# xswang/xflow

Hardware: NVIDIA H100
Metric: training examples/sec (higher is better)
Workload: dtype f32

## Files before the change

xflow_b200/csrc/kernels.cu:

```cuda
#include <cuda_runtime.h>
#include <stdint.h>
#include <stdlib.h>

#include "kernels.h"
#include "table.cuh"

__global__ void xf_k_fill(uint8_t* base, uint64_t cap, uint32_t stride, int lazy) {
  const uint64_t chunks_per_row = stride / 16;
  const uint64_t total = cap * chunks_per_row;
  for (uint64_t c = (uint64_t)blockIdx.x * blockDim.x + threadIdx.x; c < total;
       c += (uint64_t)gridDim.x * blockDim.x) {
    uint64_t r = c / chunks_per_row;
    uint32_t q = (uint32_t)(c % chunks_per_row);
    uint4 v = make_uint4(0, 0, 0, 0);
    if (q == 0) {
      v.x = 0xFFFFFFFFu; v.y = 0xFFFFFFFFu;
      if (!lazy) v.w = XF_NEG_ZERO_BITS;
    }
    *reinterpret_cast<uint4*>(base + r * stride + (uint64_t)q * 16) = v;
  }
}

template <int VEC>
__device__ __forceinline__ void xf_ldv(const float* p, float (&o)[VEC]) {
  if (VEC == 4) { float4 t = __ldcg(reinterpret_cast<const float4*>(p)); o[0] = t.x; o[1 % VEC] = t.y; o[2 % VEC] = t.z; o[3 % VEC] = t.w; }
  else if (VEC == 2) { float2 t = __ldcg(reinterpret_cast<const float2*>(p)); o[0] = t.x; o[1 % VEC] = t.y; }
  else { o[0] = __ldcg(p); }
}
template <int VEC>
__device__ __forceinline__ void xf_stv(float* p, const float (&o)[VEC]) {
  if (VEC == 4) *reinterpret_cast<float4*>(p) = make_float4(o[0], o[1 % VEC], o[2 % VEC], o[3 % VEC]);
  else if (VEC == 2) *reinterpret_cast<float2*>(p) = make_float2(o[0], o[1 % VEC]);
  else *p = o[0];
}
template <int VEC, bool SLOTG, bool STAMP>
__global__ void __launch_bounds__(256)
xf_k_update(XfTableView t, const uint32_t* __restrict__ slots, uint64_t n, int tps, double rows,
            const float* __restrict__ gw, const float* __restrict__ gv, int part,
            unsigned long long* __restrict__ live_total, const uint32_t* __restrict__ n_dev,
            const uint32_t* __restrict__ rows_dev, uint32_t extra_base, uint32_t extra_n,
            const float* __restrict__ v0_side, XfStampView sv) {
  __shared__ unsigned int s_live;
  if (threadIdx.x == 0) s_live = 0;
  __syncthreads();
  uint64_t n_head = n;
  if (n_dev != nullptr) {
    n_head = min((uint64_t)__ldg(n_dev), (uint64_t)extra_base);
    n = n_head + extra_n;
    rows = (double)__ldg(rows_dev);
  }
  unsigned int live_acc = 0;
  const int K = t.K;
  const unsigned lane = threadIdx.x & 31u;
  const uint64_t gwarp = ((uint64_t)blockIdx.x * blockDim.x + threadIdx.x) >> 5;
  const uint64_t nwarps = ((uint64_t)gridDim.x * blockDim.x) >> 5;
  const int q = (int)(lane & (unsigned)(tps - 1));
  const int gi = (int)(lane / (unsigned)tps);
  const int ngroups = 32 / tps;
  const int leader = (int)(lane & ~(unsigned)(tps - 1));
  const unsigned group_mask = (tps == 32) ? 0xffffffffu : (((1u << tps) - 1u) << leader);
  const int nchunk = K / VEC;

  for (uint64_t base = gwarp * 32; base < n; base += nwarps * 32) {
    const uint64_t e_fwd = base + lane;
    const uint64_t e_i = (SLOTG && e_fwd < n) ? (n - 1 - e_fwd) : e_fwd;
    const uint64_t e_phys = (e_i < n_head) ? e_i : (uint64_t)extra_base + (e_i - n_head);
    const uint32_t s_lane = (e_fwd < n) ? __ldcs(slots + e_phys) : 0xFFFFFFFFu;
    unsigned pend = __ballot_sync(0xffffffffu, s_lane != 0xFFFFFFFFu);
    if (live_total != nullptr && lane == 0) live_acc += __popc(pend);

    while (pend) {
      const int cnt = __popc(pend);
      const unsigned src = (gi < cnt) ? __fns(pend, 0, gi + 1) : 0u;
      const uint32_t s = __shfl_sync(0xffffffffu, s_lane, (int)src);
      const uint64_t i = __shfl_sync(0xffffffffu, (unsigned long long)e_i, (int)src);
      const uint64_t i_phys = __shfl_sync(0xffffffffu, (unsigned long long)e_phys, (int)src);
      uint8_t* rowp = (gi < cnt) ? xf_row(t, s) : nullptr;
      pend = (cnt <= ngroups) ? 0u : (pend & ~((2u << __fns(pend, 0, ngroups)) - 1u));

      const bool lat = K > 0 && (part & 2) && rowp != nullptr;
      float* vp = lat ? xf_row_v(rowp) : nullptr;
      float* nvp = lat ? xf_row_nv(rowp, K) : nullptr;
      float* zvp = lat ? xf_row_zv(rowp, K) : nullptr;
      float v0[VEC], n0[VEC], z0[VEC];
#pragma unroll
      for (int e = 0; e < VEC; ++e) { v0[e] = 0.f; n0[e] = 0.f; z0[e] = 0.f; }
      const bool has0 = lat && q < nchunk;
      if (has0) {
        xf_ldv<VEC>(vp + q * VEC, v0);
        if (t.opt == XF_OPT_FTRL) { xf_ldv<VEC>(nvp + q * VEC, n0); xf_ldv<VEC>(zvp + q * VEC, z0); }
      }
      float p0[VEC];
#pragma unroll
      for (int e = 0; e < VEC; ++e) p0[e] = 0.f;
      if (SLOTG && v0_side != nullptr && has0) {
        const uint64_t tok = (i_phys < (uint64_t)extra_base) ? i_phys : (uint64_t)__ldg(slots + i_phys + extra_n);
        xf_ldv<VEC>(v0_side + tok * (uint64_t)K + q * VEC, p0);
      }
      float ca0[VEC];
#pragma unroll
      for (int e = 0; e < VEC; ++e) ca0[e] = 0.f;
      if (SLOTG && t.canon && has0) xf_ldv<VEC>(xf_row_ca(t, rowp) + q * VEC, ca0);
      double accL = 0.0, accA = 0.0;
      if (SLOTG && has0) {
        const double2 a = __ldcg(reinterpret_cast<const double2*>(xf_row_acc(rowp, K)));
        accL = a.x;
        accA = a.y;
      }
      XfHead h;
      h.key = 0; h.flags = 0; h.w = h.n = h.z = 0.f; h.g = 0.0;
      if (q == 0 && rowp != nullptr) h = xf_load_head(rowp);
      const uint64_t key = __shfl_sync(group_mask, (unsigned long long)h.key, leader);
      const uint32_t flags = __shfl_sync(group_mask, h.flags, leader);
      if (rowp == nullptr) continue;

      if (q == 0) {
        if (!SLOTG) xf_apply_pending(t, h);
        if (part & 1) {
          const float g = SLOTG ? xf_div_rows((float)h.g, rows) : gw[i];
          xf_opt_coord(t, g, h.w, h.n, h.z);
        }
        if (SLOTG) h.g = -0.0;
        if (K > 0 && (part & 2)) h.flags |= XF_FLAG_V_READY;
        xf_store_head_t(t, rowp, h);
        if (STAMP) sv.stamp[s] = sv.now;
      }
      if (lat) {
        const bool ready = (flags & XF_FLAG_V_READY) != 0;
        for (int c = q; c < nchunk; c += tps) {
          const int k = c * VEC;
          float v[VEC], g[VEC], nn[VEC], zz[VEC];
#pragma unroll
          for (int e = 0; e < VEC; ++e) { v[e] = v0[e]; nn[e] = n0[e]; zz[e] = z0[e]; }
          if (c != q && ready) {
            xf_ldv<VEC>(vp + k, v);
            if (t.opt == XF_OPT_FTRL) { xf_ldv<VEC>(nvp + k, nn); xf_ldv<VEC>(zvp + k, zz); }
          }
          if (!ready) {
#pragma unroll
            for (int e = 0; e < VEC; ++e) { v[e] = xf_v_init(t, key, (uint32_t)(k + e)); nn[e] = 0.f; zz[e] = 0.f; }
          }
          if (SLOTG) {
            float vp0[VEC];
#pragma unroll
            for (int e = 0; e < VEC; ++e) vp0[e] = v[e];
            if (v0_side != nullptr) {
              if (c == q) {
#pragma unroll
                for (int e = 0; e < VEC; ++e) vp0[e] = p0[e];
              } else {
                const uint64_t tok = (i_phys < (uint64_t)extra_base) ? i_phys : (uint64_t)__ldg(slots + i_phys + extra_n);
                xf_ldv<VEC>(v0_side + tok * (uint64_t)K + k, vp0);
              }
            }
            if (t.canon) {
              float ca[VEC];
#pragma unroll
              for (int e = 0; e < VEC; ++e) ca[e] = ca0[e];
              if (c != q) xf_ldv<VEC>(xf_row_ca(t, rowp) + k, ca);
#pragma unroll
              for (int e = 0; e < VEC; ++e) g[e] = xf_div_rows((float)((double)ca[e] - (double)vp0[e] * accL), rows);
              const float zero[VEC] = {};
              xf_stv<VEC>(xf_row_ca(t, rowp) + k, zero);
            } else {
#pragma unroll
              for (int e = 0; e < VEC; ++e) g[e] = xf_div_rows((float)(accA - (double)vp0[e] * accL), rows);
            }
          } else {
#pragma unroll
            for (int e = 0; e < VEC; ++e) g[e] = gv[i * (uint64_t)K + k + e];
          }
          if (t.opt == XF_OPT_FTRL) {
#pragma unroll
            for (int e = 0; e < VEC; ++e) xf_ftrl_coord(t, g[e], v[e], nn[e], zz[e]);
            xf_stv<VEC>(nvp + k, nn);
            xf_stv<VEC>(zvp + k, zz);
          } else {
#pragma unroll
            for (int e = 0; e < VEC; ++e) xf_sgd_coord(t, g[e], v[e]);
          }
          xf_stv<VEC>(vp + k, v);
        }
        if (SLOTG) {
          __syncwarp(group_mask);
          if (q == 0) *reinterpret_cast<double2*>(xf_row_acc(rowp, K)) = make_double2(0.0, 0.0);
        }
      }
    }
  }
  if (live_total != nullptr) {
    if (lane == 0 && live_acc) atomicAdd(&s_live, live_acc);
    __syncthreads();
    if (threadIdx.x == 0 && s_live) atomicAdd_system(live_total, (unsigned long long)s_live);
  }
}

template <bool SLOTG>
__global__ void __launch_bounds__(256, 4)
xf_k_update_wide(XfTableView t, const uint32_t* __restrict__ slots, uint64_t n, int G, double rows,
                 const float* __restrict__ gw, const float* __restrict__ gv, int part,
                 unsigned long long* __restrict__ live_total, const uint32_t* __restrict__ n_dev,
                 const uint32_t* __restrict__ rows_dev, uint32_t extra_base, uint32_t extra_n,
                 const float* __restrict__ v0_side, XfStampView sv) {
  __shared__ unsigned int s_live;
  if (threadIdx.x == 0) s_live = 0;
  __syncthreads();
  uint64_t n_head = n;
  if (n_dev != nullptr) {
    n_head = min((uint64_t)__ldg(n_dev), (uint64_t)extra_base);
    n = n_head + extra_n;
    rows = (double)__ldg(rows_dev);
  }
  unsigned int live_acc = 0;
  const int K = t.K;
  const bool ftrl = t.opt == XF_OPT_FTRL;
  const int nV = K >> 2;
  const int units = (int)(t.stride >> 4);
  const int u_acc = 2 + nV, u_nv = u_acc + 1, u_zv = u_nv + nV;
  const unsigned lane = threadIdx.x & 31u;
  const uint64_t gwarp = ((uint64_t)blockIdx.x * blockDim.x + threadIdx.x) >> 5;
  const uint64_t nwarps = ((uint64_t)gridDim.x * blockDim.x) >> 5;
  const int q = (int)(lane & (unsigned)(G - 1));
  const int gi = (int)(lane / (unsigned)G);
  const int ngroups = 32 / G;
  const bool is_v = q >= 2 && q < 2 + nV;
  const int jv = q - 2;
  const int src_nv = is_v ? u_nv + jv : 0, src_zv = (is_v && ftrl) ? u_zv + jv : 0;
  const bool is_nv = ftrl && q >= u_nv && q < u_nv + nV, is_zv = ftrl && q >= u_zv && q < u_zv + nV;
  const int back = is_nv ? 2 + (q - u_nv) : (is_zv ? 2 + (q - u_zv) : 0);

  for (uint64_t base = gwarp * 32; base < n; base += nwarps * 32) {
    const uint64_t e_fwd = base + lane;
    const uint64_t e_i = (SLOTG && e_fwd < n) ? (n - 1 - e_fwd) : e_fwd;
    const uint64_t e_phys = (e_i < n_head) ? e_i : (uint64_t)extra_base + (e_i - n_head);
    const uint32_t s_lane = (e_fwd < n) ? __ldcs(slots + e_phys) : 0xFFFFFFFFu;
    unsigned pend = __ballot_sync(0xffffffffu, s_lane != 0xFFFFFFFFu);
    if (live_total != nullptr && lane == 0) live_acc += __popc(pend);
    while (pend) {
      const int cnt = __popc(pend);
      const unsigned src = (gi < cnt) ? __fns(pend, 0, gi + 1) : 0u;
      const uint32_t s = __shfl_sync(0xffffffffu, s_lane, (int)src);
      const uint64_t i = __shfl_sync(0xffffffffu, (unsigned long long)e_i, (int)src);
      const uint64_t i_phys = __shfl_sync(0xffffffffu, (unsigned long long)e_phys, (int)src);
      const bool live = gi < cnt;
      uint4* rowu = live ? reinterpret_cast<uint4*>(xf_row(t, s)) : nullptr;
      pend = (cnt <= ngroups) ? 0u : (pend & ~((2u << __fns(pend, 0, ngroups)) - 1u));

      uint4 u = make_uint4(0, 0, 0, 0);
      if (live && q < units) u = __ldcg(rowu + q);
      float4 side = make_float4(0.f, 0.f, 0.f, 0.f);
      if (live && is_v) {
        if (SLOTG) {
          if (v0_side != nullptr) {
            const uint64_t tok = (i_phys < (uint64_t)extra_base) ? i_phys : (uint64_t)__ldg(slots + i_phys + extra_n);
            side = __ldcg(reinterpret_cast<const float4*>(v0_side + tok * (uint64_t)K) + jv);
          }
        } else {
          side = __ldcg(reinterpret_cast<const float4*>(gv + i * (uint64_t)K) + jv);
        }
      }
      float gw_i = 0.f;
      if (!SLOTG && live && q == 1 && (part & 1)) gw_i = __ldg(gw + i);

      const uint32_t key_lo = __shfl_sync(0xffffffffu, u.x, 0, G), key_hi = __shfl_sync(0xffffffffu, u.y, 0, G);
      const uint32_t g_lo = __shfl_sync(0xffffffffu, u.z, 0, G), g_hi = __shfl_sync(0xffffffffu, u.w, 0, G);
      const uint32_t flags = __shfl_sync(0xffffffffu, u.w, 1, G);
      const uint32_t aL0 = __shfl_sync(0xffffffffu, u.x, u_acc, G), aL1 = __shfl_sync(0xffffffffu, u.y, u_acc, G);
      const uint32_t aA0 = __shfl_sync(0xffffffffu, u.z, u_acc, G), aA1 = __shfl_sync(0xffffffffu, u.w, u_acc, G);
      uint4 un, uz;
      un.x = __shfl_sync(0xffffffffu, u.x, src_nv, G); un.y = __shfl_sync(0xffffffffu, u.y, src_nv, G);
      un.z = __shfl_sync(0xffffffffu, u.z, src_nv, G); un.w = __shfl_sync(0xffffffffu, u.w, src_nv, G);
      uz.x = __shfl_sync(0xffffffffu, u.x, src_zv, G); uz.y = __shfl_sync(0xffffffffu, u.y, src_zv, G);
      uz.z = __shfl_sync(0xffffffffu, u.z, src_zv, G); uz.w = __shfl_sync(0xffffffffu, u.w, src_zv, G);
      const uint64_t key = (uint64_t)key_lo | ((uint64_t)key_hi << 32);
      const double g_acc = __longlong_as_double((long long)((uint64_t)g_lo | ((uint64_t)g_hi << 32)));
      const double accL = __longlong_as_double((long long)((uint64_t)aL0 | ((uint64_t)aL1 << 32)));
      const double accA = __longlong_as_double((long long)((uint64_t)aA0 | ((uint64_t)aA1 << 32)));
      const bool ready = (flags & XF_FLAG_V_READY) != 0;

      uint4 out = u;
      float nn[4] = {0.f, 0.f, 0.f, 0.f}, zz[4] = {0.f, 0.f, 0.f, 0.f};
      if (q == 0 && SLOTG) { out.z = 0u; out.w = XF_NEG_ZERO_BITS; }
      if (q == 1) {
        float w = __uint_as_float(u.x), nw = __uint_as_float(u.y), zw = __uint_as_float(u.z);
        if (part & 1) {
          const float g = SLOTG ? xf_div_rows((float)g_acc, rows) : gw_i;
          xf_opt_coord(t, g, w, nw, zw);
        }
        out.x = __float_as_uint(w); out.y = __float_as_uint(nw); out.z = __float_as_uint(zw);
        out.w = u.w | XF_FLAG_V_READY;
      }
      if (is_v) {
        float v[4] = {__uint_as_float(u.x), __uint_as_float(u.y), __uint_as_float(u.z), __uint_as_float(u.w)};
        nn[0] = __uint_as_float(un.x); nn[1] = __uint_as_float(un.y); nn[2] = __uint_as_float(un.z); nn[3] = __uint_as_float(un.w);
        zz[0] = __uint_as_float(uz.x); zz[1] = __uint_as_float(uz.y); zz[2] = __uint_as_float(uz.z); zz[3] = __uint_as_float(uz.w);
        if (!ready) {
#pragma unroll
          for (int e = 0; e < 4; ++e) { v[e] = xf_v_init(t, key, (uint32_t)(4 * jv + e)); nn[e] = 0.f; zz[e] = 0.f; }
        }
        float g[4];
        if (SLOTG) {
          const float p[4] = {side.x, side.y, side.z, side.w};
#pragma unroll
          for (int e = 0; e < 4; ++e) g[e] = xf_div_rows((float)(accA - (double)(v0_side != nullptr ? p[e] : v[e]) * accL), rows);
        } else {
          g[0] = side.x; g[1] = side.y; g[2] = side.z; g[3] = side.w;
        }
        if (ftrl) {
#pragma unroll 1
          for (int e = 0; e < 4; ++e) xf_ftrl_coord(t, g[e], v[e], nn[e], zz[e]);
        } else {
#pragma unroll
          for (int e = 0; e < 4; ++e) xf_sgd_coord(t, g[e], v[e]);
        }
        out = make_uint4(__float_as_uint(v[0]), __float_as_uint(v[1]), __float_as_uint(v[2]), __float_as_uint(v[3]));
      }
      uint4 bn, bz;
      bn.x = __shfl_sync(0xffffffffu, __float_as_uint(nn[0]), back, G); bn.y = __shfl_sync(0xffffffffu, __float_as_uint(nn[1]), back, G);
      bn.z = __shfl_sync(0xffffffffu, __float_as_uint(nn[2]), back, G); bn.w = __shfl_sync(0xffffffffu, __float_as_uint(nn[3]), back, G);
      bz.x = __shfl_sync(0xffffffffu, __float_as_uint(zz[0]), back, G); bz.y = __shfl_sync(0xffffffffu, __float_as_uint(zz[1]), back, G);
      bz.z = __shfl_sync(0xffffffffu, __float_as_uint(zz[2]), back, G); bz.w = __shfl_sync(0xffffffffu, __float_as_uint(zz[3]), back, G);
      if (is_nv) out = bn;
      if (is_zv) out = bz;
      if (q == u_acc && SLOTG) out = make_uint4(0, 0, 0, 0);
      if (live && q < units) rowu[q] = out;
      if (SLOTG && live && q == 0 && sv.stamp != nullptr) sv.stamp[s] = sv.now;
    }
  }
  if (live_total != nullptr) {
    if (lane == 0 && live_acc) atomicAdd(&s_live, live_acc);
    __syncthreads();
    if (threadIdx.x == 0 && s_live) atomicAdd_system(live_total, (unsigned long long)s_live);
  }
}

template <bool INSERT>
__global__ void xf_k_probe(XfTableView t, const uint64_t* __restrict__ keys, uint64_t n,
                           uint32_t* __restrict__ slots, float* __restrict__ w_out, XfStampView sv) {
  for (uint64_t i = (uint64_t)blockIdx.x * blockDim.x + threadIdx.x; i < n;
       i += (uint64_t)gridDim.x * blockDim.x) {
    XfHead h;
    h.w = 0.f;
    int64_t s = xf_probe<INSERT, true>(t, keys[i], &h, &sv);
    slots[i] = s >= 0 ? (uint32_t)s : 0xFFFFFFFFu;
    if (w_out) {
      if (s >= 0) xf_apply_pending(t, h);
      w_out[i] = s >= 0 ? h.w : 0.f;
    }
  }
}

__global__ void xf_k_gather_v(XfTableView t, const uint32_t* __restrict__ slots, const uint64_t* __restrict__ keys,
                              uint64_t n, float* __restrict__ v_out) {
  const int K = t.K;
  const uint64_t total = n * (uint64_t)K;
  for (uint64_t x = (uint64_t)blockIdx.x * blockDim.x + threadIdx.x; x < total;
       x += (uint64_t)gridDim.x * blockDim.x) {
    const uint64_t i = x / K;
    const int k = (int)(x % K);
    const uint32_t s = slots[i];
    float v = 0.f;
    if (s != 0xFFFFFFFFu) {
      const uint8_t* rowp = xf_row(t, s);
      const uint32_t flags = __ldcg(reinterpret_cast<const uint32_t*>(rowp + XF_OFF_FLAGS));
      v = (flags & XF_FLAG_V_READY) ? __ldcg(reinterpret_cast<const float*>(rowp + 32) + k)
                                    : xf_v_init(t, keys[i], (uint32_t)k);
    }
    v_out[x] = v;
  }
}

__global__ void xf_k_import(XfTableView t, const uint32_t* __restrict__ slots, uint64_t n,
                            const float* w, const float* nw, const float* zw, const float* v,
                            const float* nv, const float* zv) {
  const int K = t.K;
  const uint64_t per = (uint64_t)K + 1;
  const uint64_t total = n * per;
  for (uint64_t x = (uint64_t)blockIdx.x * blockDim.x + threadIdx.x; x < total;
       x += (uint64_t)gridDim.x * blockDim.x) {
    const uint64_t i = x / per;
    const int c = (int)(x % per);
    const uint32_t s = slots[i];
    if (s == 0xFFFFFFFFu) continue;
    uint8_t* rowp = xf_row(t, s);
    if (c == 0) {
      if (w) {
        if (t.lazy) {
          XfHead h;
          h.key = *reinterpret_cast<const uint64_t*>(rowp);
          h.w = w[i]; h.n = nw ? nw[i] : 0.f; h.z = zw ? zw[i] : 0.f; h.flags = 0u; h.g = 0.0;
          xf_lazy_store(t, rowp, h, true);
        } else {
          *reinterpret_cast<float2*>(rowp + XF_OFF_STATE) = make_float2(w[i], nw ? nw[i] : 0.f);
          *reinterpret_cast<float*>(rowp + XF_OFF_STATE + 8) = zw ? zw[i] : 0.f;
          *reinterpret_cast<unsigned long long*>(rowp + 8) = XF_NEG_ZERO_BITS64;
        }
      }
      if (v && K > 0) *reinterpret_cast<uint32_t*>(rowp + XF_OFF_FLAGS) = XF_FLAG_V_READY;
    } else if (v) {
      const int k = c - 1;
      xf_row_v(rowp)[k] = v[i * K + k];
      if (k == 0) *reinterpret_cast<double2*>(xf_row_acc(rowp, K)) = make_double2(0.0, 0.0);
      if (t.opt == XF_OPT_FTRL) {
        xf_row_nv(rowp, K)[k] = nv ? nv[i * K + k] : 0.f;
        xf_row_zv(rowp, K)[k] = zv ? zv[i * K + k] : 0.f;
      }
    }
  }
}

__global__ void xf_k_export(XfTableView t, const uint32_t* __restrict__ slots, const uint64_t* __restrict__ keys,
                            uint64_t n, float* w, float* nw, float* zw, float* v, float* nv, float* zv,
                            uint8_t* present) {
  const int K = t.K;
  const uint64_t per = (uint64_t)K + 1;
  const uint64_t total = n * per;
  for (uint64_t x = (uint64_t)blockIdx.x * blockDim.x + threadIdx.x; x < total;
       x += (uint64_t)gridDim.x * blockDim.x) {
    const uint64_t i = x / per;
    const int c = (int)(x % per);
    const uint32_t s = slots[i];
    const bool have = s != 0xFFFFFFFFu;
    const uint8_t* rowp = have ? xf_row(t, s) : nullptr;
    if (c == 0) {
      XfHead h;
      h.w = h.n = h.z = 0.f;
      if (have) {
        h = xf_load_head(rowp);
        xf_apply_pending(t, h);
      }
      if (present) present[i] = have ? 1 : 0;
      if (w) w[i] = h.w;
      if (nw) nw[i] = h.n;
      if (zw) zw[i] = h.z;
    } else if (v) {
      const int k = c - 1;
      float vv = 0.f, nn = 0.f, zz = 0.f;
      if (have) {
        const uint32_t flags = __ldcg(reinterpret_cast<const uint32_t*>(rowp + XF_OFF_FLAGS));
        if (flags & XF_FLAG_V_READY) {
          vv = __ldcg(reinterpret_cast<const float*>(rowp + 32) + k);
          if (t.opt == XF_OPT_FTRL) {
            nn = __ldcg(xf_row_nv(const_cast<uint8_t*>(rowp), K) + k);
            zz = __ldcg(xf_row_zv(const_cast<uint8_t*>(rowp), K) + k);
          }
        } else {
          vv = xf_v_init(t, keys[i], (uint32_t)k);
        }
      }
      v[i * K + k] = vv;
      if (nv) nv[i * K + k] = nn;
      if (zv) zv[i * K + k] = zz;
    }
  }
}

__global__ void xf_k_rehash(XfTableView src, XfTableView dst, XfKeep keep, const uint32_t* __restrict__ src_stamp,
                            uint32_t* __restrict__ dst_stamp) {
  const uint64_t cap = src.mask + 1;
  const uint32_t chunks = src.stride / 16;
  for (uint64_t r = (uint64_t)blockIdx.x * blockDim.x + threadIdx.x; r < cap;
       r += (uint64_t)gridDim.x * blockDim.x) {
    const uint8_t* srow = xf_row(src, r);
    uint4 a = *reinterpret_cast<const uint4*>(srow);
    uint64_t key = (uint64_t)a.x | ((uint64_t)a.y << 32);
    if (key == XF_EMPTY_KEY) continue;
    const uint32_t stamp = src_stamp != nullptr ? src_stamp[r] : 0u;
    if (src_stamp != nullptr && !xf_keeps(keep, stamp, key)) continue;
    XfHead h;
    int64_t s = xf_probe<true>(dst, key, &h);
    if (s < 0) continue;
    uint8_t* drow = xf_row(dst, (uint64_t)s);
    *reinterpret_cast<uint2*>(drow + 8) = make_uint2(a.z, a.w);
    for (uint32_t c = 1; c < chunks; ++c)
      *reinterpret_cast<uint4*>(drow + 16 * c) = *reinterpret_cast<const uint4*>(srow + 16 * c);
    if (dst_stamp != nullptr) dst_stamp[s] = stamp;
  }
}

__global__ void xf_k_list_keys(XfTableView t, uint64_t* keys_out, unsigned long long* count, uint64_t max_out) {
  const uint64_t cap = t.mask + 1;
  for (uint64_t r = (uint64_t)blockIdx.x * blockDim.x + threadIdx.x; r < cap;
       r += (uint64_t)gridDim.x * blockDim.x) {
    const uint64_t key = *reinterpret_cast<const uint64_t*>(xf_row(t, r));
    if (key == XF_EMPTY_KEY) continue;
    unsigned long long idx = atomicAdd(count, 1ull);
    if (idx < max_out) keys_out[idx] = key;
  }
}

static int g_sm_count = 0;
int xf_sms() {
  if (g_sm_count == 0) {
    int dev = 0;
    cudaGetDevice(&dev);
    cudaDeviceGetAttribute(&g_sm_count, cudaDevAttrMultiProcessorCount, dev);
    if (g_sm_count <= 0) g_sm_count = 132;
  }
  return g_sm_count;
}
int xf_grid_for(uint64_t work_items, int block, int blocks_per_sm) {
  uint64_t want = (work_items + block - 1) / block;
  uint64_t cap = (uint64_t)xf_sms() * blocks_per_sm;
  if (want < 1) want = 1;
  return (int)(want < cap ? want : cap);
}

int xf_vec_for(int K) { return K <= 0 ? 1 : (K % 4 == 0 ? 4 : (K % 2 == 0 ? 2 : 1)); }
int xf_tps_for(int K) {
  if (K <= 0) return 1;
  int chunks = K / xf_vec_for(K);
  int tps = 1;
  while (tps < chunks && tps < 32) tps <<= 1;
  return tps;
}

void xf_launch_fill(const XfTableView& t, cudaStream_t st) {
  uint64_t cap = t.mask + 1;
  uint64_t total = cap * (t.stride / 16);
  xf_k_fill<<<xf_grid_for(total, 256, 16), 256, 0, st>>>(t.base, cap, t.stride, t.lazy);
}

template <bool SLOTG, bool STAMP = false>
static void xf_launch_update_t(const XfTableView& t, const uint32_t* slots, uint64_t n, double rows,
                               const float* gw, const float* gv, int part, unsigned long long* live_total,
                               cudaStream_t st, const uint32_t* n_dev = nullptr, const uint32_t* rows_dev = nullptr,
                               uint32_t extra_base = 0, uint32_t extra_n = 0, const float* v0_side = nullptr,
                               XfStampView sv = XfStampView{nullptr, 0u}) {
  static const bool wide_on = [] { const char* e = getenv("XFLOW_UPDATE_WIDE"); return e && *e == '1'; }();
  if (wide_on && !t.canon && t.K > 0 && (t.K & 3) == 0 && t.stride <= 512 && (part & 2)) {
    int G = 1;
    while (G < (int)(t.stride >> 4)) G <<= 1;
    const int grid = xf_grid_for(n * (uint64_t)G, 256, 8);
    xf_k_update_wide<SLOTG><<<grid, 256, 0, st>>>(t, slots, n, G, rows, gw, gv, part, live_total, n_dev, rows_dev,
                                                   extra_base, extra_n, v0_side, sv);
    return;
  }
  const int tps = xf_tps_for(t.K);
  const int grid = xf_grid_for(n * (uint64_t)tps, 256, 8);
#define XF_UPD_ARGS t, slots, n, tps, rows, gw, gv, part, live_total, n_dev, rows_dev, extra_base, extra_n, v0_side, sv
  switch (xf_vec_for(t.K)) {
    case 4: xf_k_update<4, SLOTG, STAMP><<<grid, 256, 0, st>>>(XF_UPD_ARGS); break;
    case 2: xf_k_update<2, SLOTG, STAMP><<<grid, 256, 0, st>>>(XF_UPD_ARGS); break;
    default: xf_k_update<1, SLOTG, STAMP><<<grid, 256, 0, st>>>(XF_UPD_ARGS); break;
  }
#undef XF_UPD_ARGS
}

void xf_launch_update_touched_dev(const XfTableView& t, const uint32_t* touched, uint64_t work_bound,
                                  const uint32_t* n_dev, const uint32_t* rows_dev, uint32_t extra_base,
                                  uint32_t extra_n, const float* v0_side, unsigned long long* unique_total,
                                  cudaStream_t st) {
  xf_launch_update_t<true>(t, touched, work_bound + extra_n, 1.0, nullptr, nullptr, 3, unique_total, st, n_dev, rows_dev,
                           extra_base, extra_n, v0_side);
}

__global__ void xf_k_flush_pending(XfTableView t) {
  const uint64_t cap = t.mask + 1;
  for (uint64_t r = (uint64_t)blockIdx.x * blockDim.x + threadIdx.x; r < cap; r += (uint64_t)gridDim.x * blockDim.x) {
    uint8_t* rowp = xf_row(t, r);
    XfHead h = xf_load_head(rowp);
    if (h.key == XF_EMPTY_KEY || !xf_lazy_has_pending(h)) continue;
    xf_apply_pending(t, h);
    xf_lazy_store(t, rowp, h);
  }
}
void xf_launch_flush_pending(const XfTableView& t, cudaStream_t st) {
  xf_k_flush_pending<<<xf_grid_for(t.mask + 1, 256, 8), 256, 0, st>>>(t);
}

void xf_launch_update_touched(const XfTableView& t, const uint32_t* touched, uint64_t nnz, double rows,
                              unsigned long long* unique_total, const XfStampView& sv, cudaStream_t st) {
  if (nnz == 0) return;
  if (sv.stamp)
    xf_launch_update_t<true, true>(t, touched, nnz, rows, nullptr, nullptr, 3, unique_total, st, nullptr, nullptr, 0, 0,
                                   nullptr, sv);
  else
    xf_launch_update_t<true>(t, touched, nnz, rows, nullptr, nullptr, 3, unique_total, st);
}

void xf_launch_update_pushed(const XfTableView& t, const uint32_t* slots, uint64_t n, const float* gw,
                             const float* gv, cudaStream_t st) {
  if (n == 0) return;
  int part = (gw ? 1 : 0) | (gv ? 2 : 0);
  xf_launch_update_t<false>(t, slots, n, 1.0, gw, gv, part, nullptr, st);
}

void xf_launch_probe(const XfTableView& t, const uint64_t* keys, uint64_t n, bool insert, uint32_t* slots,
                     float* w_out, cudaStream_t st, const XfStampView& sv) {
  if (n == 0) return;
  const int grid = xf_grid_for(n, 256, 8);
  if (insert) xf_k_probe<true><<<grid, 256, 0, st>>>(t, keys, n, slots, w_out, sv);
  else xf_k_probe<false><<<grid, 256, 0, st>>>(t, keys, n, slots, w_out, sv);
}

void xf_launch_gather_v(const XfTableView& t, const uint32_t* slots, const uint64_t* keys, uint64_t n,
                        float* v_out, cudaStream_t st) {
  if (n == 0 || t.K == 0) return;
  xf_k_gather_v<<<xf_grid_for(n * t.K, 256, 8), 256, 0, st>>>(t, slots, keys, n, v_out);
}

void xf_launch_import(const XfTableView& t, const uint32_t* slots, uint64_t n, const float* w, const float* nw,
                      const float* zw, const float* v, const float* nv, const float* zv, cudaStream_t st) {
  if (n == 0) return;
  xf_k_import<<<xf_grid_for(n * (t.K + 1), 256, 8), 256, 0, st>>>(t, slots, n, w, nw, zw, v, nv, zv);
}

void xf_launch_export(const XfTableView& t, const uint32_t* slots, const uint64_t* keys, uint64_t n, float* w,
                      float* nw, float* zw, float* v, float* nv, float* zv, uint8_t* present, cudaStream_t st) {
  if (n == 0) return;
  xf_k_export<<<xf_grid_for(n * (t.K + 1), 256, 8), 256, 0, st>>>(t, slots, keys, n, w, nw, zw, v, nv, zv, present);
}

void xf_launch_rehash(const XfTableView& src, const XfTableView& dst, const XfKeep& keep, const uint32_t* src_stamp,
                      uint32_t* dst_stamp, cudaStream_t st) {
  xf_k_rehash<<<xf_grid_for(src.mask + 1, 256, 8), 256, 0, st>>>(src, dst, keep, src_stamp, dst_stamp);
}

void xf_launch_list_keys(const XfTableView& t, uint64_t* keys_out, unsigned long long* count, uint64_t max_out,
                         cudaStream_t st) {
  xf_k_list_keys<<<xf_grid_for(t.mask + 1, 256, 8), 256, 0, st>>>(t, keys_out, count, max_out);
}
```

Measured before the change: 83.62 million.

## Add warp-cooperative row update kernel staging several rows in shared memory

Adds a new update kernel for SGD slot-gathered updates. Each warp compacts the live slots with a ballot and keeps several rows in flight at once, loading them with vector loads into shared memory. It then updates the coordinates from the shared copy and writes the rows back whole. This is meant to raise memory-level parallelism and give coalesced row access compared with the per-thread-group update path. The new kernel is selected by default when the shape conditions match, so it adds a separate code path that must stay in sync with the existing update semantics.

```diff
diff --git a/xflow_b200/csrc/kernels.cu b/xflow_b200/csrc/kernels.cu
--- a/xflow_b200/csrc/kernels.cu
+++ b/xflow_b200/csrc/kernels.cu
@@ -325,6 +325,109 @@
       if (q == u_acc && SLOTG) out = make_uint4(0, 0, 0, 0);
       if (live && q < units) rowu[q] = out;
       if (SLOTG && live && q == 0 && sv.stamp != nullptr) sv.stamp[s] = sv.now;
+    }
+  }
+  if (live_total != nullptr) {
+    if (lane == 0 && live_acc) atomicAdd(&s_live, live_acc);
+    __syncthreads();
+    if (threadIdx.x == 0 && s_live) atomicAdd_system(live_total, (unsigned long long)s_live);
+  }
+}
+
+#define XF_ROWS_IN_FLIGHT 4
+template <int R, bool STAMP>
+__global__ void __launch_bounds__(256, 4)
+xf_k_update_rows(XfTableView t, const uint32_t* __restrict__ slots, uint64_t n, int G, double rows,
+                 unsigned long long* __restrict__ live_total, XfStampView sv) {
+  __shared__ unsigned int s_live;
+  __shared__ __align__(16) uint4 s_row[8][R][32];
+  if (threadIdx.x == 0) s_live = 0;
+  __syncthreads();
+  unsigned int live_acc = 0;
+  const int K = t.K;
+  const bool ftrl = t.opt == XF_OPT_FTRL;
+  const int units = (int)(t.stride >> 4);
+  const int w_acc = (int)(xf_acc_off(K) >> 2);
+  const int w_nv = w_acc + 4, w_zv = w_nv + K;
+  const int per_row = K + 1;
+  const unsigned lane = threadIdx.x & 31u;
+  const int wib = (int)(threadIdx.x >> 5);
+  const uint64_t gwarp = ((uint64_t)blockIdx.x * blockDim.x + threadIdx.x) >> 5;
+  const uint64_t nwarps = ((uint64_t)gridDim.x * blockDim.x) >> 5;
+  const int q = (int)(lane & (unsigned)(G - 1));
+  const int gi = (int)(lane / (unsigned)G);
+  const int ngroups = 32 / G;
+  const int take = ngroups * R;
+  uint4 (*buf)[32] = s_row[wib];
+  uint32_t* gw0 = reinterpret_cast<uint32_t*>(&buf[0][gi * G]);
+
+  for (uint64_t base = gwarp * 32; base < n; base += nwarps * 32) {
+    const uint64_t e_fwd = base + lane;
+    const uint64_t e_i = (e_fwd < n) ? (n - 1 - e_fwd) : e_fwd;
+    const uint32_t s_lane = (e_fwd < n) ? __ldcs(slots + e_i) : 0xFFFFFFFFu;
+    unsigned pend = __ballot_sync(0xffffffffu, s_lane != 0xFFFFFFFFu);
+    if (live_total != nullptr && lane == 0) live_acc += __popc(pend);
+    while (pend) {
+      const int cnt = __popc(pend);
+      uint32_t s[R];
+      unsigned live = 0u;
+#pragma unroll
+      for (int r = 0; r < R; ++r) {
+        const int e = r * ngroups + gi;
+        const unsigned src = (e < cnt) ? __fns(pend, 0, e + 1) : 0u;
+        s[r] = __shfl_sync(0xffffffffu, s_lane, (int)src);
+        if (e < cnt) live |= 1u << r;
+      }
+      pend = (cnt <= take) ? 0u : (pend & ~((2u << __fns(pend, 0, take)) - 1u));
+      uint4 u[R];
+#pragma unroll
+      for (int r = 0; r < R; ++r) {
+        u[r] = make_uint4(0, 0, 0, 0);
+        if (((live >> r) & 1u) && q < units) u[r] = __ldcg(reinterpret_cast<const uint4*>(xf_row(t, s[r])) + q);
+      }
+#pragma unroll
+      for (int r = 0; r < R; ++r) buf[r][lane] = u[r];
+      __syncwarp();
+      for (int x = q; x < R * per_row; x += G) {
+        const int r = x / per_row, c = x - r * per_row;
+        if (!((live >> r) & 1u)) continue;
+        uint32_t* rw = gw0 + r * 128;
+        float* rf = reinterpret_cast<float*>(rw);
+        int iw = 4, in = 5, iz = 6;
+        if (c < K) { iw = 8 + c; in = w_nv + c; iz = w_zv + c; }
+        float w = rf[iw], nn = ftrl ? rf[in] : 0.f, zz = ftrl ? rf[iz] : 0.f;
+        float g;
+        if (c < K) {
+          if (!(rw[7] & XF_FLAG_V_READY)) {
+            const uint64_t key = (uint64_t)rw[0] | ((uint64_t)rw[1] << 32);
+            w = xf_v_init(t, key, (uint32_t)c);
+            nn = 0.f;
+            zz = 0.f;
+          }
+          const double accL = __hiloint2double((int)rw[w_acc + 1], (int)rw[w_acc]);
+          const double accA = __hiloint2double((int)rw[w_acc + 3], (int)rw[w_acc + 2]);
+          g = xf_div_rows((float)(accA - (double)w * accL), rows);
+        } else {
+          g = xf_div_rows((float)__hiloint2double((int)rw[3], (int)rw[2]), rows);
+        }
+        xf_opt_coord(t, g, w, nn, zz);
+        rf[iw] = w;
+        if (ftrl) { rf[in] = nn; rf[iz] = zz; }
+      }
+      __syncwarp();
+#pragma unroll
+      for (int r = 0; r < R; ++r) {
+        if (!((live >> r) & 1u)) continue;
+        if (q < units) {
+          uint4 o = buf[r][lane];
+          if (q == 0) { o.z = 0u; o.w = XF_NEG_ZERO_BITS; }
+          if (q == 1) o.w |= XF_FLAG_V_READY;
+          if (q == (w_acc >> 2)) o = make_uint4(0, 0, 0, 0);
+          reinterpret_cast<uint4*>(xf_row(t, s[r]))[q] = o;
+        }
+        if (STAMP && q == 0) sv.stamp[s[r]] = sv.now;
+      }
+      __syncwarp();
     }
   }
   if (live_total != nullptr) {
@@ -528,9 +631,15 @@
                                uint32_t extra_base = 0, uint32_t extra_n = 0, const float* v0_side = nullptr,
                                XfStampView sv = XfStampView{nullptr, 0u}) {
   static const bool wide_on = [] { const char* e = getenv("XFLOW_UPDATE_WIDE"); return e && *e == '1'; }();
-  if (wide_on && !t.canon && t.K > 0 && (t.K & 3) == 0 && t.stride <= 512 && (part & 2)) {
-    int G = 1;
-    while (G < (int)(t.stride >> 4)) G <<= 1;
+  const bool row_shape = !t.canon && t.K > 0 && (t.K & 3) == 0 && t.stride <= 512 && (part & 2);
+  int G = 1;
+  while (G < (int)(t.stride >> 4)) G <<= 1;
+  if (SLOTG && row_shape && t.opt == XF_OPT_SGD && !wide_on && part == 3 && n_dev == nullptr && v0_side == nullptr) {
+    const int grid = xf_grid_for(n * (uint64_t)G, 256, 8);
+    xf_k_update_rows<XF_ROWS_IN_FLIGHT, STAMP><<<grid, 256, 0, st>>>(t, slots, n, G, rows, live_total, sv);
+    return;
+  }
+  if (wide_on && row_shape) {
     const int grid = xf_grid_for(n * (uint64_t)G, 256, 8);
     xf_k_update_wide<SLOTG><<<grid, 256, 0, st>>>(t, slots, n, G, rows, gw, gv, part, live_total, n_dev, rows_dev,
                                                    extra_base, extra_n, v0_side, sv);
```

Result: no change. 83.58 million (median of 6 runs) (-0.0%).

## Stage touched rows into shared memory via cp.async pipeline for optimizer update

Applied to the files above, without the earlier changes.

Replaces the env-gated wide update kernel with a new row-tiled kernel for the touched-slot update path. Each warp copies up to R full embedding rows into a 3-stage shared-memory ring with cp.async, updates per-coordinate state in shared memory, then writes the rows back coalesced. The aim is to overlap the random row gathers with compute and to get coalesced 16-byte loads and stores. In exchange it adds 48KB of dynamic shared memory per block, which can limit occupancy, calls cudaFuncSetAttribute on every launch, and drops the n_dev/v0_side variants for this path.

```diff
diff --git a/xflow_b200/csrc/kernels.cu b/xflow_b200/csrc/kernels.cu
--- a/xflow_b200/csrc/kernels.cu
+++ b/xflow_b200/csrc/kernels.cu
@@ -1,6 +1,5 @@
 #include <cuda_runtime.h>
 #include <stdint.h>
-#include <stdlib.h>
 
 #include "kernels.h"
 #include "table.cuh"
@@ -195,137 +194,133 @@
   }
 }
 
-template <bool SLOTG>
+#define XF_ROWS_TILE_UNITS 128
+#define XF_ROWS_STAGES 3
+
+struct XfRowsWalk {
+  uint64_t base;
+  uint32_t s_lane;
+  unsigned pend;
+};
+__device__ __forceinline__ int xf_rows_next(XfRowsWalk& w, const uint32_t* __restrict__ slots, uint64_t n,
+                                            uint64_t step, int R, unsigned int& live_acc, bool count, uint32_t& s_row) {
+  const unsigned lane = threadIdx.x & 31u;
+  while (w.pend == 0u) {
+    w.base += step;
+    if (w.base >= n) return 0;
+    const uint64_t e_fwd = w.base + lane;
+    w.s_lane = (e_fwd < n) ? __ldcs(slots + (n - 1 - e_fwd)) : 0xFFFFFFFFu;
+    w.pend = __ballot_sync(0xffffffffu, w.s_lane != 0xFFFFFFFFu);
+    if (count && lane == 0) live_acc += __popc(w.pend);
+  }
+  const int cnt = __popc(w.pend);
+  const int nr = cnt < R ? cnt : R;
+  s_row = __shfl_sync(0xffffffffu, w.s_lane, ((int)lane < nr) ? (int)__fns(w.pend, 0, lane + 1) : 0);
+  w.pend = (cnt <= R) ? 0u : (w.pend & ~((2u << __fns(w.pend, 0, R)) - 1u));
+  return nr;
+}
+__device__ __forceinline__ void xf_cp_async16(void* smem, const void* gmem) {
+  asm volatile("cp.async.cg.shared.global [%0], [%1], 16;" ::"r"((uint32_t)__cvta_generic_to_shared(smem)), "l"(gmem)
+               : "memory");
+}
+
+template <bool STAMP>
 __global__ void __launch_bounds__(256, 4)
-xf_k_update_wide(XfTableView t, const uint32_t* __restrict__ slots, uint64_t n, int G, double rows,
-                 const float* __restrict__ gw, const float* __restrict__ gv, int part,
-                 unsigned long long* __restrict__ live_total, const uint32_t* __restrict__ n_dev,
-                 const uint32_t* __restrict__ rows_dev, uint32_t extra_base, uint32_t extra_n,
-                 const float* __restrict__ v0_side, XfStampView sv) {
+xf_k_update_rows(XfTableView t, const uint32_t* __restrict__ slots, uint64_t n, int R, double rows,
+                 unsigned long long* __restrict__ live_total, XfStampView sv) {
+  extern __shared__ uint4 s_tiles[];
   __shared__ unsigned int s_live;
   if (threadIdx.x == 0) s_live = 0;
   __syncthreads();
-  uint64_t n_head = n;
-  if (n_dev != nullptr) {
-    n_head = min((uint64_t)__ldg(n_dev), (uint64_t)extra_base);
-    n = n_head + extra_n;
-    rows = (double)__ldg(rows_dev);
-  }
   unsigned int live_acc = 0;
-  const int K = t.K;
+  const int K = t.K, D = K + 1;
   const bool ftrl = t.opt == XF_OPT_FTRL;
-  const int nV = K >> 2;
-  const int units = (int)(t.stride >> 4);
-  const int u_acc = 2 + nV, u_nv = u_acc + 1, u_zv = u_nv + nV;
+  const uint32_t stride = t.stride;
+  const int units = (int)(stride >> 4);
+  const uint32_t acc = xf_acc_off(K);
+  const int u_acc = (int)(acc >> 4);
   const unsigned lane = threadIdx.x & 31u;
-  const uint64_t gwarp = ((uint64_t)blockIdx.x * blockDim.x + threadIdx.x) >> 5;
-  const uint64_t nwarps = ((uint64_t)gridDim.x * blockDim.x) >> 5;
-  const int q = (int)(lane & (unsigned)(G - 1));
-  const int gi = (int)(lane / (unsigned)G);
-  const int ngroups = 32 / G;
-  const bool is_v = q >= 2 && q < 2 + nV;
-  const int jv = q - 2;
-  const int src_nv = is_v ? u_nv + jv : 0, src_zv = (is_v && ftrl) ? u_zv + jv : 0;
-  const bool is_nv = ftrl && q >= u_nv && q < u_nv + nV, is_zv = ftrl && q >= u_zv && q < u_zv + nV;
-  const int back = is_nv ? 2 + (q - u_nv) : (is_zv ? 2 + (q - u_zv) : 0);
-
-  for (uint64_t base = gwarp * 32; base < n; base += nwarps * 32) {
-    const uint64_t e_fwd = base + lane;
-    const uint64_t e_i = (SLOTG && e_fwd < n) ? (n - 1 - e_fwd) : e_fwd;
-    const uint64_t e_phys = (e_i < n_head) ? e_i : (uint64_t)extra_base + (e_i - n_head);
-    const uint32_t s_lane = (e_fwd < n) ? __ldcs(slots + e_phys) : 0xFFFFFFFFu;
-    unsigned pend = __ballot_sync(0xffffffffu, s_lane != 0xFFFFFFFFu);
-    if (live_total != nullptr && lane == 0) live_acc += __popc(pend);
-    while (pend) {
-      const int cnt = __popc(pend);
-      const unsigned src = (gi < cnt) ? __fns(pend, 0, gi + 1) : 0u;
-      const uint32_t s = __shfl_sync(0xffffffffu, s_lane, (int)src);
-      const uint64_t i = __shfl_sync(0xffffffffu, (unsigned long long)e_i, (int)src);
-      const uint64_t i_phys = __shfl_sync(0xffffffffu, (unsigned long long)e_phys, (int)src);
-      const bool live = gi < cnt;
-      uint4* rowu = live ? reinterpret_cast<uint4*>(xf_row(t, s)) : nullptr;
-      pend = (cnt <= ngroups) ? 0u : (pend & ~((2u << __fns(pend, 0, ngroups)) - 1u));
-
-      uint4 u = make_uint4(0, 0, 0, 0);
-      if (live && q < units) u = __ldcg(rowu + q);
-      float4 side = make_float4(0.f, 0.f, 0.f, 0.f);
-      if (live && is_v) {
-        if (SLOTG) {
-          if (v0_side != nullptr) {
-            const uint64_t tok = (i_phys < (uint64_t)extra_base) ? i_phys : (uint64_t)__ldg(slots + i_phys + extra_n);
-            side = __ldcg(reinterpret_cast<const float4*>(v0_side + tok * (uint64_t)K) + jv);
-          }
-        } else {
-          side = __ldcg(reinterpret_cast<const float4*>(gv + i * (uint64_t)K) + jv);
+  uint4* tiles = s_tiles + (threadIdx.x >> 5) * (XF_ROWS_STAGES * XF_ROWS_TILE_UNITS);
+  int it_r[4], it_u[4];
+#pragma unroll
+  for (int j = 0; j < 4; ++j) {
+    const int it = (int)lane + 32 * j;
+    it_r[j] = it < R * units ? it / units : 32;
+    it_u[j] = it < R * units ? it - it_r[j] * units : 0;
+  }
+  const uint64_t step = ((uint64_t)gridDim.x * blockDim.x) >> 5 << 5;
+  XfRowsWalk walk{(((uint64_t)blockIdx.x * blockDim.x + threadIdx.x) >> 5 << 5) - step, 0u, 0u};
+  const bool count = live_total != nullptr;
+
+  auto fetch = [&](int nr, uint32_t s_row, uint4* tile) {
+#pragma unroll
+    for (int j = 0; j < 4; ++j) {
+      const uint32_t s = __shfl_sync(0xffffffffu, s_row, it_r[j] & 31);
+      if (it_r[j] < nr) xf_cp_async16(tile + lane + 32 * j, reinterpret_cast<const uint4*>(xf_row(t, s)) + it_u[j]);
+    }
+    asm volatile("cp.async.commit_group;" ::: "memory");
+  };
+  uint32_t s_cur, s1;
+  int nr = xf_rows_next(walk, slots, n, step, R, live_acc, count, s_cur);
+  fetch(nr, s_cur, tiles);
+  int nr1 = xf_rows_next(walk, slots, n, step, R, live_acc, count, s1);
+  fetch(nr1, s1, tiles + XF_ROWS_TILE_UNITS);
+  for (int buf = 0; nr > 0; buf = (buf == XF_ROWS_STAGES - 1) ? 0 : buf + 1) {
+    uint32_t s2;
+    const int nr2 = xf_rows_next(walk, slots, n, step, R, live_acc, count, s2);
+    fetch(nr2, s2, tiles + ((buf + 2) % XF_ROWS_STAGES) * XF_ROWS_TILE_UNITS);
+    asm volatile("cp.async.wait_group 2;" ::: "memory");
+    __syncwarp();
+
+    uint4* tile = tiles + buf * XF_ROWS_TILE_UNITS;
+    uint8_t* tb = reinterpret_cast<uint8_t*>(tile);
+    for (int c = (int)lane; c < nr * D; c += 32) {
+      const int r = c / D, k = c - r * D - 1;
+      uint8_t* row = tb + r * stride;
+      float* wp = reinterpret_cast<float*>(row + (k < 0 ? XF_OFF_STATE : 32 + 4 * k));
+      float* np = k < 0 ? wp + 1 : reinterpret_cast<float*>(row + acc + 16) + k;
+      float* zp = k < 0 ? wp + 2 : np + K;
+      float w = *wp, nn = 0.f, zz = 0.f;
+      if (ftrl) { nn = *np; zz = *zp; }
+      float g;
+      if (k < 0) {
+        g = xf_div_rows((float)*reinterpret_cast<const double*>(row + 8), rows);
+      } else {
+        if (!(*reinterpret_cast<const uint32_t*>(row + XF_OFF_FLAGS) & XF_FLAG_V_READY)) {
+          w = xf_v_init(t, *reinterpret_cast<const uint64_t*>(row), (uint32_t)k);
+          nn = 0.f;
+          zz = 0.f;
         }
-      }
-      float gw_i = 0.f;
-      if (!SLOTG && live && q == 1 && (part & 1)) gw_i = __ldg(gw + i);
-
-      const uint32_t key_lo = __shfl_sync(0xffffffffu, u.x, 0, G), key_hi = __shfl_sync(0xffffffffu, u.y, 0, G);
-      const uint32_t g_lo = __shfl_sync(0xffffffffu, u.z, 0, G), g_hi = __shfl_sync(0xffffffffu, u.w, 0, G);
-      const uint32_t flags = __shfl_sync(0xffffffffu, u.w, 1, G);
-      const uint32_t aL0 = __shfl_sync(0xffffffffu, u.x, u_acc, G), aL1 = __shfl_sync(0xffffffffu, u.y, u_acc, G);
-      const uint32_t aA0 = __shfl_sync(0xffffffffu, u.z, u_acc, G), aA1 = __shfl_sync(0xffffffffu, u.w, u_acc, G);
-      uint4 un, uz;
-      un.x = __shfl_sync(0xffffffffu, u.x, src_nv, G); un.y = __shfl_sync(0xffffffffu, u.y, src_nv, G);
-      un.z = __shfl_sync(0xffffffffu, u.z, src_nv, G); un.w = __shfl_sync(0xffffffffu, u.w, src_nv, G);
-      uz.x = __shfl_sync(0xffffffffu, u.x, src_zv, G); uz.y = __shfl_sync(0xffffffffu, u.y, src_zv, G);
-      uz.z = __shfl_sync(0xffffffffu, u.z, src_zv, G); uz.w = __shfl_sync(0xffffffffu, u.w, src_zv, G);
-      const uint64_t key = (uint64_t)key_lo | ((uint64_t)key_hi << 32);
-      const double g_acc = __longlong_as_double((long long)((uint64_t)g_lo | ((uint64_t)g_hi << 32)));
-      const double accL = __longlong_as_double((long long)((uint64_t)aL0 | ((uint64_t)aL1 << 32)));
-      const double accA = __longlong_as_double((long long)((uint64_t)aA0 | ((uint64_t)aA1 << 32)));
-      const bool ready = (flags & XF_FLAG_V_READY) != 0;
-
-      uint4 out = u;
-      float nn[4] = {0.f, 0.f, 0.f, 0.f}, zz[4] = {0.f, 0.f, 0.f, 0.f};
-      if (q == 0 && SLOTG) { out.z = 0u; out.w = XF_NEG_ZERO_BITS; }
-      if (q == 1) {
-        float w = __uint_as_float(u.x), nw = __uint_as_float(u.y), zw = __uint_as_float(u.z);
-        if (part & 1) {
-          const float g = SLOTG ? xf_div_rows((float)g_acc, rows) : gw_i;
-          xf_opt_coord(t, g, w, nw, zw);
-        }
-        out.x = __float_as_uint(w); out.y = __float_as_uint(nw); out.z = __float_as_uint(zw);
-        out.w = u.w | XF_FLAG_V_READY;
-      }
-      if (is_v) {
-        float v[4] = {__uint_as_float(u.x), __uint_as_float(u.y), __uint_as_float(u.z), __uint_as_float(u.w)};
-        nn[0] = __uint_as_float(un.x); nn[1] = __uint_as_float(un.y); nn[2] = __uint_as_float(un.z); nn[3] = __uint_as_float(un.w);
-        zz[0] = __uint_as_float(uz.x); zz[1] = __uint_as_float(uz.y); zz[2] = __uint_as_float(uz.z); zz[3] = __uint_as_float(uz.w);
-        if (!ready) {
-#pragma unroll
-          for (int e = 0; e < 4; ++e) { v[e] = xf_v_init(t, key, (uint32_t)(4 * jv + e)); nn[e] = 0.f; zz[e] = 0.f; }
-        }
-        float g[4];
-        if (SLOTG) {
-          const float p[4] = {side.x, side.y, side.z, side.w};
-#pragma unroll
-          for (int e = 0; e < 4; ++e) g[e] = xf_div_rows((float)(accA - (double)(v0_side != nullptr ? p[e] : v[e]) * accL), rows);
-        } else {
-          g[0] = side.x; g[1] = side.y; g[2] = side.z; g[3] = side.w;
-        }
-        if (ftrl) {
-#pragma unroll 1
-          for (int e = 0; e < 4; ++e) xf_ftrl_coord(t, g[e], v[e], nn[e], zz[e]);
-        } else {
-#pragma unroll
-          for (int e = 0; e < 4; ++e) xf_sgd_coord(t, g[e], v[e]);
-        }
-        out = make_uint4(__float_as_uint(v[0]), __float_as_uint(v[1]), __float_as_uint(v[2]), __float_as_uint(v[3]));
-      }
-      uint4 bn, bz;
-      bn.x = __shfl_sync(0xffffffffu, __float_as_uint(nn[0]), back, G); bn.y = __shfl_sync(0xffffffffu, __float_as_uint(nn[1]), back, G);
-      bn.z = __shfl_sync(0xffffffffu, __float_as_uint(nn[2]), back, G); bn.w = __shfl_sync(0xffffffffu, __float_as_uint(nn[3]), back, G);
-      bz.x = __shfl_sync(0xffffffffu, __float_as_uint(zz[0]), back, G); bz.y = __shfl_sync(0xffffffffu, __float_as_uint(zz[1]), back, G);
-      bz.z = __shfl_sync(0xffffffffu, __float_as_uint(zz[2]), back, G); bz.w = __shfl_sync(0xffffffffu, __float_as_uint(zz[3]), back, G);
-      if (is_nv) out = bn;
-      if (is_zv) out = bz;
-      if (q == u_acc && SLOTG) out = make_uint4(0, 0, 0, 0);
-      if (live && q < units) rowu[q] = out;
-      if (SLOTG && live && q == 0 && sv.stamp != nullptr) sv.stamp[s] = sv.now;
-    }
+        const double2 a = *reinterpret_cast<const double2*>(row + acc);
+        g = xf_div_rows((float)(a.y - (double)w * a.x), rows);
+      }
+      if (ftrl) {
+        xf_ftrl_coord(t, g, w, nn, zz);
+        *np = nn;
+        *zp = zz;
+      } else {
+        xf_sgd_coord(t, g, w);
+      }
+      *wp = w;
+    }
+    __syncwarp();
+
+#pragma unroll
+    for (int j = 0; j < 4; ++j) {
+      const uint32_t s = __shfl_sync(0xffffffffu, s_cur, it_r[j] & 31);
+      if (it_r[j] < nr) {
+        uint4 o = tile[lane + 32 * j];
+        if (it_u[j] == 0) { o.z = 0u; o.w = XF_NEG_ZERO_BITS; }
+        if (it_u[j] == 1) o.w |= XF_FLAG_V_READY;
+        if (it_u[j] == u_acc) o = make_uint4(0u, 0u, 0u, 0u);
+        reinterpret_cast<uint4*>(xf_row(t, s))[it_u[j]] = o;
+      }
+    }
+    if (STAMP && (int)lane < nr) sv.stamp[s_cur] = sv.now;
+    nr = nr1;
+    s_cur = s1;
+    nr1 = nr2;
+    s1 = s2;
   }
   if (live_total != nullptr) {
     if (lane == 0 && live_acc) atomicAdd(&s_live, live_acc);
@@ -527,15 +522,6 @@
                                cudaStream_t st, const uint32_t* n_dev = nullptr, const uint32_t* rows_dev = nullptr,
                                uint32_t extra_base = 0, uint32_t extra_n = 0, const float* v0_side = nullptr,
                                XfStampView sv = XfStampView{nullptr, 0u}) {
-  static const bool wide_on = [] { const char* e = getenv("XFLOW_UPDATE_WIDE"); return e && *e == '1'; }();
-  if (wide_on && !t.canon && t.K > 0 && (t.K & 3) == 0 && t.stride <= 512 && (part & 2)) {
-    int G = 1;
-    while (G < (int)(t.stride >> 4)) G <<= 1;
-    const int grid = xf_grid_for(n * (uint64_t)G, 256, 8);
-    xf_k_update_wide<SLOTG><<<grid, 256, 0, st>>>(t, slots, n, G, rows, gw, gv, part, live_total, n_dev, rows_dev,
-                                                   extra_base, extra_n, v0_side, sv);
-    return;
-  }
   const int tps = xf_tps_for(t.K);
   const int grid = xf_grid_for(n * (uint64_t)tps, 256, 8);
 #define XF_UPD_ARGS t, slots, n, tps, rows, gw, gv, part, live_total, n_dev, rows_dev, extra_base, extra_n, v0_side, sv
@@ -572,6 +558,19 @@
 void xf_launch_update_touched(const XfTableView& t, const uint32_t* touched, uint64_t nnz, double rows,
                               unsigned long long* unique_total, const XfStampView& sv, cudaStream_t st) {
   if (nnz == 0) return;
+  if (t.K > 0 && !t.canon && t.stride <= 512) {
+    const int R = min(16, XF_ROWS_TILE_UNITS / (int)(t.stride >> 4));
+    const int grid = xf_grid_for(nnz, 256, 8);
+    const int smem = 8 * XF_ROWS_STAGES * XF_ROWS_TILE_UNITS * 16;
+    if (sv.stamp) {
+      cudaFuncSetAttribute(xf_k_update_rows<true>, cudaFuncAttributeMaxDynamicSharedMemorySize, smem);
+      xf_k_update_rows<true><<<grid, 256, smem, st>>>(t, touched, nnz, R, rows, unique_total, sv);
+    } else {
+      cudaFuncSetAttribute(xf_k_update_rows<false>, cudaFuncAttributeMaxDynamicSharedMemorySize, smem);
+      xf_k_update_rows<false><<<grid, 256, smem, st>>>(t, touched, nnz, R, rows, unique_total, sv);
+    }
+    return;
+  }
   if (sv.stamp)
     xf_launch_update_t<true, true>(t, touched, nnz, rows, nullptr, nullptr, 3, unique_total, st, nullptr, nullptr, 0, 0,
                                    nullptr, sv);
```

After: 83.61 million before, 83.42 million after, median of 6. Within noise of the previous version (-0.2%).
